# steineggerlab/unicore

Hardware: AMD Instinct MI355X
Metric: 3Di alignments/sec (cluster path) (higher is better)
Workload: dtype u16

## Files before the change

### include/unicore_cluster.h

```cpp
#ifndef UNICORE_CLUSTER_H
#define UNICORE_CLUSTER_H
#include <stddef.h>
#include <stdint.h>
#ifdef __cplusplus
extern "C" {
#endif

#define UC_OK 0
#define UC_ERR_GENERIC 1
#define UC_ERR_ARGS 2
#define UC_ERR_IO 3
#define UC_ERR_DEVICE 4

typedef struct uc_opts {
    uint32_t struct_size;
    int32_t threads;
    int32_t verbosity;
    int32_t device;
    int32_t num_gpus;
    const char *cluster_options;
    const char *data_dir;
} uc_opts;

#define UC_ABI_VERSION 9
// ... 103 lines not shown
#define UC_COMM_ID_BYTES 128
int uc_comm_unique_id(uint8_t id[UC_COMM_ID_BYTES]);
int uc_comm_create(const uint8_t id[UC_COMM_ID_BYTES], int32_t rank, int32_t world, int32_t device, uc_comm **out);
void uc_comm_destroy(uc_comm *c);
int uc_comm_info(const uc_comm *c, int32_t *nccl_ranks, int32_t *nccl_rank, int32_t *device);
int uc_engine_cluster_step(uc_engine *e, uc_comm *comm, int32_t target_shards, uint32_t *assign, uint64_t *n_alignments);

int uc_engine_align(uc_engine *e, uint32_t qbegin, uint32_t qend);
int uc_engine_alns_get(const uc_engine *e, uint32_t qbegin, uint32_t qend, uc_aln *out);
int uc_engine_edges_size(const uc_engine *e, uint64_t *n_edges);
int uc_engine_edges_get(const uc_engine *e, uint32_t *edges );

int uc_engine_stats(const uc_engine *e, uc_stats *out);
void uc_engine_reset_stats(uc_engine *e);
int uc_engine_td_onchip(const uc_engine *e, uint64_t *out );

int uc_engine_linclust_pairs(uc_engine *e, int32_t m, int32_t install, uint32_t *out_pairs, uint64_t cap, uint64_t *n_out);

int uc_setcover(uint32_t n, const uint32_t *edges, uint64_t n_edges, uint32_t *assign);
int uc_engine_setcover(uc_engine *e, const uint32_t *edges, uint64_t n_edges, uint32_t *assign);
int uc_cluster_graph(uint32_t n, const uint32_t *edges, uint64_t n_edges, const uint32_t *len, int32_t mode, uint32_t *assign);
int uc_engine_cluster_graph(uc_engine *e, int32_t mode, const uint32_t *edges, uint64_t n_edges, uint32_t *assign);
int uc_engine_reassign(uc_engine *e, const uint32_t *assign_in, uint32_t *assign_out, uint8_t *rejected_out, uint64_t counts[4]);
int uc_write_cluster_db(const char *out_cluster_db, uint32_t n, const uint32_t *assign);

#define UC_NO_GENE 0xffffffffu
int uc_profile_count(uint64_t n_rows, const uint32_t *group, const uint32_t *gene, uint32_t n_groups, uint32_t n_genes, const uint64_t *sp_off,
                     const uint32_t *sp, uint32_t n_species, uint32_t threshold, uint32_t *single, uint32_t *multiple, uint8_t *core,
                     uint64_t *core_off, uint32_t *core_gene, uint32_t *core_species, uint32_t *full);
int uc_profile_count_dev(int32_t device, uint64_t n_rows, const uint32_t *group, const uint32_t *gene, uint32_t n_groups, uint32_t n_genes,
// ... 114 lines not shown
```

### unicore_amd/__init__.py

```python
import ctypes as C
import os

import numpy as np

_HERE = os.path.dirname(os.path.abspath(__file__))
LIB_PATH = os.path.join(_HERE, "libunicore_cluster.so")

UC_OK, UC_ERR_GENERIC, UC_ERR_ARGS, UC_ERR_IO, UC_ERR_DEVICE = 0, 1, 2, 3, 4
NSTAGE = 8
PHASES = ("prefilter", "exchange_lists_to_home", "merge_at_home", "exchange_pairs_to_owner", "install_owned", "gapped", "edge_gather", "rank0_serial_cover")
STAGES = ("load", "index", "kmer", "ungapped", "select", "gapped", "setcover", "output")


class UcOpts(C.Structure):
    _fields_ = [("struct_size", C.c_uint32), ("threads", C.c_int32), ("verbosity", C.c_int32), ("device", C.c_int32),
                ("num_gpus", C.c_int32), ("cluster_options", C.c_char_p), ("data_dir", C.c_char_p)]


class UcStats(C.Structure):
    _fields_ = [(n, C.c_uint64) for n in (
        "n_seqs", "n_residues", "n_index_entries", "n_sim_kmers", "n_kmer_hits", "n_candidates", "n_prefilter_hits",
        "n_gapped_alignments", "n_start_alignments", "n_pk_reruns", "n_edges", "n_clusters", "cells_fwd", "cells_rev", "cells_start")] + [
        ("algorithmic_bytes", C.c_uint64 * NSTAGE), ("stage_seconds", C.c_double * NSTAGE),
        ("sw_kernel_ms", C.c_double), ("sw_kernel_launches", C.c_uint64), ("sw_algorithmic_bytes", C.c_uint64),
# ... 43 lines not shown
HIT_DTYPE = np.dtype([("target", "<u4"), ("score", "<i4"), ("diag", "<i4")])
ALN_DTYPE = np.dtype([(n, "<i4") for n in ("score", "score_rev", "corrected", "qstart", "qend", "tstart", "tend",
                                            "aln_len", "idents", "pass_evalue", "accepted", "gap_opens")])

SYMBOLS = (
    "uc_cluster", "uc_createtsv", "uc_rmdb", "uc_search", "uc_convertalis", "uc_last_error", "uc_version", "uc_check_options",
    "uc_option_arity", "uc_release_scratch", "uc_createdb", "uc_t5_load", "uc_t5_free", "uc_t5_encode", "uc_t5_get_stats", "uc_comm_unique_id", "uc_comm_create", "uc_comm_destroy", "uc_comm_info", "uc_engine_cluster_step",
    "uc_engine_create", "uc_engine_destroy", "uc_engine_load_db", "uc_engine_set_db", "uc_engine_num_seqs",
    "uc_engine_prefilter", "uc_engine_prefilter_range", "uc_engine_hits_size", "uc_engine_hits_get", "uc_engine_hits_get_range", "uc_engine_hits_set", "uc_engine_hits_merge",
    "uc_engine_hits_export_dev", "uc_engine_hits_import_dev", "uc_engine_setcover",
    "uc_hits_merge", "uc_engine_align", "uc_engine_alns_get", "uc_engine_edges_size", "uc_engine_edges_get",
    "uc_engine_stats", "uc_engine_reset_stats", "uc_setcover", "uc_write_cluster_db",
    "uc_engine_ungapped_batch", "uc_engine_ungapped_select", "uc_engine_ungapped_all", "uc_engine_sw_batch", "uc_engine_sw_pass", "uc_engine_sw_pass2", "uc_engine_backtraces_size", "uc_engine_backtraces_get",
    "uc_backtrace_render", "uc_format_output_check", "uc_engine_tb_emit_pass", "uc_abi_version", "uc_stats_size", "uc_set_round_hook",
    "uc_t5_gemm_variant", "uc_t5_kernel_gemm", "uc_t5_kernel_rmsnorm", "uc_t5_kernel_attention", "uc_t5_kernel_cnn_head", "uc_t5_bias_table",
    "uc_cluster_graph", "uc_engine_cluster_graph", "uc_engine_reassign", "uc_engine_td_onchip", "uc_engine_linclust_pairs",
    "uc_profile_count", "uc_profile_count_dev", "uc_profile",
    "uc_msa_center", "uc_msa_center_dev", "uc_msa_star", "uc_msa_star_dev", "uc_msa_filter", "uc_msa_filter_dev", "uc_tree",
    "uc_nj_counts", "uc_nj_counts_dev", "uc_nj_distances", "uc_nj_join", "uc_nj_join_dev", "uc_nj_newick", "uc_nj_geometry", "uc_tree_infer",
    "uc_nj_boot_columns", "uc_nj_boot_counts", "uc_nj_boot_counts_dev", "uc_nj_join_batch", "uc_nj_join_batch_dev", "uc_nj_support", "uc_nj_newick_support",
    "uc_nj_boot_geometry", "uc_tree_infer_boot",
)
NO_GENE = 0xFFFFFFFF
ABI_VERSION = 9
ROUND_HOOK = C.CFUNCTYPE(None, C.c_void_p, C.c_int32, C.c_uint32, C.POINTER(C.c_uint32), C.c_int32, C.c_void_p)

_lib = None


class UcError(RuntimeError):
    def __init__(self, code, msg):
# ... 45 lines not shown
    L.uc_engine_hits_get_range.argtypes = [vp, u32, u32, vp, vp]
    L.uc_engine_hits_set.argtypes = [vp, vp, vp]
    L.uc_engine_hits_merge.argtypes = [vp, C.c_int, C.POINTER(vp), C.POINTER(vp)]
    L.uc_engine_hits_export_dev.argtypes = [vp, vp, vp, vp, vp]
    L.uc_engine_setcover.argtypes = [vp, vp, u64, vp]
    L.uc_engine_hits_import_dev.argtypes = [vp, u64, vp, vp, vp, vp, u32, u32, C.POINTER(u64)]
    L.uc_hits_merge.argtypes = [u32, i32, C.c_int, C.POINTER(vp), C.POINTER(vp), vp, vp, u64, C.POINTER(u64)]
    L.uc_engine_align.argtypes = [vp, u32, u32]
    L.uc_engine_alns_get.argtypes = [vp, u32, u32, vp]
    L.uc_engine_edges_size.argtypes = [vp, C.POINTER(u64)]
    L.uc_engine_edges_get.argtypes = [vp, vp]
    L.uc_engine_stats.argtypes = [vp, C.POINTER(UcStats)]
    L.uc_engine_reset_stats.argtypes = [vp]
    L.uc_engine_reset_stats.restype = None
    L.uc_engine_td_onchip.argtypes = [vp, C.POINTER(C.c_uint64)]
    L.uc_engine_linclust_pairs.argtypes = [vp, i32, i32, vp, u64, C.POINTER(u64)]
    L.uc_setcover.argtypes = [u32, vp, u64, vp]
    L.uc_cluster_graph.argtypes = [u32, vp, u64, vp, i32, vp]
    L.uc_engine_cluster_graph.argtypes = [vp, i32, vp, u64, vp]
    L.uc_engine_reassign.argtypes = [vp, vp, vp, vp, vp]
    L.uc_write_cluster_db.argtypes = [C.c_char_p, u32, vp]
    L.uc_profile_count.argtypes = [u64, vp, vp, u32, u32, vp, vp, u32, u32] + [vp] * 7
    L.uc_profile_count_dev.argtypes = [i32, u64, vp, vp, u32, u32, vp, vp, u32, u32] + [vp] * 7
    L.uc_profile.argtypes = [C.c_char_p, C.c_char_p, C.c_char_p, u32, C.POINTER(UcOpts)]
    L.uc_msa_center.argtypes = [u32, vp, vp, vp]
    L.uc_msa_center_dev.argtypes = [i32, u32, vp, vp, vp]
    L.uc_msa_star.argtypes = [u32, vp, vp, u32] + [vp] * 8 + [vp, vp, vp, u64, vp, vp, u64, vp]
    L.uc_msa_star_dev.argtypes = [i32] + L.uc_msa_star.argtypes
    L.uc_msa_filter.argtypes = [u32, vp, vp, vp, u32, vp, vp, vp]
    L.uc_msa_filter_dev.argtypes = [i32] + L.uc_msa_filter.argtypes
# ... 655 lines not shown

    def edges(self):
        ne = C.c_uint64()
        _check(lib().uc_engine_edges_size(self._h, C.byref(ne)))
        e = np.zeros((max(ne.value, 1), 2), np.uint32)
        _check(lib().uc_engine_edges_get(self._h, e.ctypes.data))
        return e[: ne.value]

    def stats(self):
        st = UcStats()
        _check(lib().uc_engine_stats(self._h, C.byref(st)))
        d = st.as_dict()
        td = (C.c_uint64 * 4)()
        _check(lib().uc_engine_td_onchip(self._h, td))
        d["td_onchip_queries"], d["td_onchip_keys"] = int(td[0]), int(td[2])
        return d

    def reset_stats(self):
        lib().uc_engine_reset_stats(self._h)

    def ungapped(self, q, t, diag):
        q = np.ascontiguousarray(q, np.uint32); t = np.ascontiguousarray(t, np.uint32)
        diag = np.ascontiguousarray(diag, np.int32)
        out = np.zeros(len(q), np.int32)
        _check(lib().uc_engine_ungapped_batch(self._h, len(q), q.ctypes.data, t.ctypes.data, diag.ctypes.data, out.ctypes.data))
        return out

    def ungapped_select(self, q, t, diag, min_score):
        q = np.ascontiguousarray(q, np.uint32); t = np.ascontiguousarray(t, np.uint32)
        diag = np.ascontiguousarray(diag, np.int32)
# ... 66 lines not shown
```

### unicore_amd/csrc/uc_capi.cpp

```cpp
#include <sys/stat.h>

#include <algorithm>
#include <cmath>
#include <cstdlib>
#include <cstring>
#include <fstream>
#include <memory>

#include "uc_engine.h"
#include "uc_files.h"
#include "uc_multi.h"
#include "uc_t5.h"
#include "uc_workflow.h"

using namespace uc;

struct uc_comm {
    Comm c;
};
struct uc_t5 {
    T5Model m;
};

namespace {
// ... 316 lines not shown
        if (!h.empty()) { require(edges, "edges"); memcpy(edges, h.data(), h.size() * 4); }
    });
}

int uc_engine_stats(const uc_engine *e, uc_stats *out) {
    return guard([&] { require(e, "engine"); require(out, "out"); *out = e->e->stats; });
}

void uc_engine_reset_stats(uc_engine *e) {
    if (!e || !e->e) return;
    uc_stats &s = e->e->stats;
    const uint64_t ns = s.n_seqs, nr = s.n_residues;
    memset(&s, 0, sizeof s);
    s.n_seqs = ns; s.n_residues = nr;
    for (uint64_t &x : e->e->td_onchip) x = 0;
}

int uc_engine_td_onchip(const uc_engine *e, uint64_t *out) {
    return guard([&] { require(e, "engine"); require(out, "out"); for (int i = 0; i < 4; i++) out[i] = e->e->td_onchip[i]; });
}

int uc_engine_linclust_pairs(uc_engine *e, int32_t m, int32_t install, uint32_t *out_pairs, uint64_t cap, uint64_t *n_out) {
    return guard([&] {
        require(e, "engine"); require(n_out, "n_out");
        if (m > 1000) fail(UC_ERR_ARGS, "uc_engine_linclust_pairs: m must be <= 0 (the engine's --kmer-per-seq) or in [1,1000]");
        if (install != 0 && install != 1) fail(UC_ERR_ARGS, "uc_engine_linclust_pairs: install must be 0 or 1");
        if (cap && !install) require(out_pairs, "out_pairs");
        const int mo = m > 0 ? m : 0;
        if (install) { *n_out = e->e->linclust_hits(mo); return; }
        const std::vector<uint32_t> pr = e->e->linclust_pairs(mo);
// ... 460 lines not shown
```

### unicore_amd/csrc/uc_device.h

```cpp
#pragma once
#include <hip/hip_runtime.h>

#include <atomic>
#include <cstdint>

namespace uc {

struct PerDeviceOnce {
    std::atomic<uint64_t> mask{0};
    template <typename F>
    void operator()(F &&f) {
        int d = 0;
        (void)hipGetDevice(&d);
        const uint64_t bit = 1ull << (d & 63);
        if (!(mask.load(std::memory_order_acquire) & bit)) { f(); mask.fetch_or(bit, std::memory_order_release); }
    }
};

struct DeviceDb {
    uint32_t n = 0;
    const uint8_t *s3 = nullptr, *sa = nullptr;
    const uint16_t *lt = nullptr;
    const uint32_t *off = nullptr;
    const uint32_t *len = nullptr;
// ... 7 lines not shown

struct SwArgs {
    DeviceDb db;
    const SwTask *tasks;
    const uint32_t *pt;
    const int32_t *pqe, *pte;
    const int32_t *pqs = nullptr, *pts = nullptr;
    uint8_t *tbm = nullptr;
    const unsigned long long *tboff = nullptr;
    int tb_band = 0;
    const int32_t *pscore = nullptr;
    int32_t *oscore, *oqe, *ote;
    int open, ext;
    uint32_t tb_diag = 1u, tb_ident = 0u, tb_open = 1u, tb_ext = 1u;
    int32_t *oqe2 = nullptr, *ote2 = nullptr;
};

constexpr int SW_MAX_ROWS = 2048;

struct TbBand { int nl, dlo, dhi; };
__host__ __device__ inline TbBand tb_band_of(int qs, int qe, int tl, int G, int R, int W) {
    TbBand b;
    const int d0 = qs, d1 = qe - (tl - 1);
    b.dlo = (d0 < d1 ? d0 : d1) - W;
    b.dhi = (d0 < d1 ? d1 : d0) + W;
    const int nl = (b.dhi - b.dlo + R - 1) / (R + 1) + 1;
    b.nl = (W <= 0 || nl >= G) ? G : nl;
    return b;
}

// ... 14 lines not shown
__device__ __forceinline__ void block_add2(unsigned long long va, unsigned long long vb, T *da, T *db) {
    __shared__ unsigned long long part[2][16];
    for (int o = 32; o > 0; o >>= 1) { va += __shfl_down(va, o, 64); vb += __shfl_down(vb, o, 64); }
    if ((threadIdx.x & 63) == 0) { part[0][threadIdx.x >> 6] = va; part[1][threadIdx.x >> 6] = vb; }
    __syncthreads();
    if (threadIdx.x == 0) {
        unsigned long long sa = 0, sb = 0;
        for (uint32_t w = 0; w < (blockDim.x + 63) >> 6; w++) { sa += part[0][w]; sb += part[1][w]; }
        if (sa) atomicAdd(da, (T)sa);
        if (sb) atomicAdd(db, (T)sb);
    }
}
#endif

void launch_sw_class(int G, int R, int mode, const SwArgs &a, uint32_t n_tasks, hipStream_t s);
void launch_sw_pk_class(int G, int R, int mode, const SwArgs &a, uint32_t n_tasks, hipStream_t s);
constexpr uint32_t SW_LONG_TASK_PAIRS = 8;
size_t sw_long_work_ints(int mode, uint32_t n_pairs, uint32_t max_len, uint32_t *stride);
void launch_sw_long(int mode, const SwArgs &a, uint32_t n_tasks, uint32_t pair_base, int32_t *work, uint32_t stride, hipStream_t s);
void launch_ungapped(const DeviceDb &db, uint64_t n, const uint32_t *q, const uint32_t *t, const int32_t *diag,
                     int32_t *score, unsigned long long *overlap_sum , hipStream_t s);
void launch_comp_bias(const DeviceDb &db, int scale_milli, int8_t *out, hipStream_t s);
void launch_db_pad(uint32_t n, const uint32_t *off, const uint32_t *len, const uint32_t *cur ,
                   const uint64_t *roff, const uint8_t *r3, const uint8_t *ra,
                   uint64_t total, uint8_t *s3, uint8_t *sa, uint16_t *lt, hipStream_t s);

}
```

### unicore_amd/csrc/uc_engine.h

```cpp
#pragma once
#include <hip/hip_runtime.h>

#include <algorithm>
#include <atomic>
#include <chrono>
#include <cstdint>
#include <cstdio>
#include <cstdlib>
#include <memory>
#include <mutex>
#include <string>
#include <utility>
#include <vector>

#include "uc_common.h"
#include "uc_db.h"
#include "uc_device.h"
#include "uc_options.h"
#include "unicore_cluster.h"

namespace uc {

struct OomRelief { bool (*fn)(void *) = nullptr; void *ctx = nullptr; };
inline OomRelief &oom_relief_slot() { static thread_local OomRelief r; return r; }
// ... 215 lines not shown
    void clear_edges() { edges.clear(); n_edges_dev = 0; edges_on_host = true; }
    const std::vector<uint32_t> &host_edges();

    uc_stats stats{};

    explicit Engine(const Params &pp, int dev);
    ~Engine();
    void upload_db(bool keep_raw = false);
    void upload_sub_db(const std::vector<uint32_t> &cur, const std::vector<uint64_t> &full_off);
    uint64_t plan_db_layout();
    void finish_db_install(struct Timer &tm);
    void prefilter(uint32_t tbegin, uint32_t tend, uint32_t qbegin = 0, uint32_t qend = UINT32_MAX);
    void prefilter_cells(uint32_t tbegin, uint32_t tend, const std::vector<std::pair<uint32_t, uint32_t>> &others);
    PrefilterScratch *pre = nullptr;
    AlignScratch *aln = nullptr;
    uint64_t td_onchip[4] = {0, 0, 0, 0};
    uint64_t last_align_hits = 0;
    void drop_scratch();
    bool relieve_pressure(int stage);
    int stage_frames[3] = {0, 0, 0};
    struct PressureScope {
        OomRelief saved;
        struct Ctx { Engine *e; int stage; } ctx;
        PressureScope(Engine &E, int stage) : saved(oom_relief_slot()), ctx{&E, stage} {
            E.stage_frames[stage]++;
            oom_relief_slot() = OomRelief{[](void *c) { return ((Ctx *)c)->e->relieve_pressure(((Ctx *)c)->stage); }, &ctx};
        }
        ~PressureScope() { oom_relief_slot() = saved; ctx.e->stage_frames[ctx.stage]--; }
        PressureScope(const PressureScope &) = delete;
        PressureScope &operator=(const PressureScope &) = delete;
// ... 51 lines not shown
```

### unicore_amd/csrc/uc_sw.hip

```cpp
#include "uc_sw_impl.hpp"

namespace uc {

void launch_sw_class_m0(int G, int R, const SwArgs &a, uint32_t n_tasks, hipStream_t s);
void launch_sw_class_m1(int G, int R, const SwArgs &a, uint32_t n_tasks, hipStream_t s);
void launch_sw_class_m2(int G, int R, const SwArgs &a, uint32_t n_tasks, hipStream_t s);
void launch_sw_class_m3(int G, int R, const SwArgs &a, uint32_t n_tasks, hipStream_t s);

void launch_sw_class(int G, int R, int mode, const SwArgs &a, uint32_t n_tasks, hipStream_t s) {
    if (n_tasks == 0) return;
    if (mode == 0) launch_sw_class_m0(G, R, a, n_tasks, s);
    else if (mode == 1) launch_sw_class_m1(G, R, a, n_tasks, s);
    else if (mode == 2) launch_sw_class_m2(G, R, a, n_tasks, s);
    else launch_sw_class_m3(G, R, a, n_tasks, s);
}

void launch_sw_pk_class_m0(int G, int R, const SwArgs &a, uint32_t n_tasks, hipStream_t s);
void launch_sw_pk_class_m1(int G, int R, const SwArgs &a, uint32_t n_tasks, hipStream_t s);
void launch_sw_pk_class_m2(int G, int R, const SwArgs &a, uint32_t n_tasks, hipStream_t s);
void launch_sw_pk_class_m4(int G, int R, const SwArgs &a, uint32_t n_tasks, hipStream_t s);
void launch_sw_pk_class_m6(int G, int R, const SwArgs &a, uint32_t n_tasks, hipStream_t s);
void launch_sw_pk_class_m7(int G, int R, const SwArgs &a, uint32_t n_tasks, hipStream_t s);
void launch_sw_pk_class(int G, int R, int mode, const SwArgs &a, uint32_t n_tasks, hipStream_t s) {
    if (n_tasks == 0) return;
    if (mode == 0) launch_sw_pk_class_m0(G, R, a, n_tasks, s);
    else if (mode == 1) launch_sw_pk_class_m1(G, R, a, n_tasks, s);
    else if (mode == 2) launch_sw_pk_class_m2(G, R, a, n_tasks, s);
    else if (mode == 4) launch_sw_pk_class_m4(G, R, a, n_tasks, s);
    else if (mode == 6) launch_sw_pk_class_m6(G, R, a, n_tasks, s);
    else launch_sw_pk_class_m7(G, R, a, n_tasks, s);
}

__global__ void __launch_bounds__(256) db_pad_kernel(uint32_t n, const uint32_t *off, const uint32_t *len, const uint32_t *cur, const uint64_t *roff, const uint8_t *r3,
                                                     const uint8_t *ra, uint64_t total, uint8_t *s3, uint8_t *sa, uint16_t *lt) {
    for (uint64_t p = (uint64_t)blockIdx.x * 256 + threadIdx.x; p < total + 16; p += (uint64_t)gridDim.x * 256) {
        if (p < 16) { lt[p] = (uint16_t)SW_PADPACK; continue; }
        const uint64_t q = p - 16;
        uint8_t c3 = 20, ca = 20;
        uint16_t pair = (uint16_t)SW_PADPACK;
        if (n) {
            uint32_t lo = 0, hi = n;
            while (hi - lo > 1) {
                const uint32_t mid = lo + ((hi - lo) >> 1);
                if (off[mid] <= q) lo = mid; else hi = mid;
            }
// ... 121 lines not shown
```

### unicore_amd/csrc/uc_sw_pk_impl.hpp

```cpp
#pragma once
#include <hip/hip_runtime.h>

#include "uc_device.h"
#include "uc_sw_impl.hpp"

namespace uc {

constexpr int SW_PK_OVF = 0x7C00 - 256;

typedef uint16_t u16x2_t __attribute__((ext_vector_type(2)));
typedef uint32_t u32x4_u __attribute__((ext_vector_type(4), aligned(4)));
typedef uint32_t u32x2_u __attribute__((ext_vector_type(2), aligned(4)));
typedef const uint32_t __attribute__((address_space(4))) *sw_cu32p;
__device__ __forceinline__ u16x2_t pk_v(uint32_t x) { return __builtin_bit_cast(u16x2_t, x); }
__device__ __forceinline__ uint32_t pk_u(u16x2_t v) { return __builtin_bit_cast(uint32_t, v); }
__device__ __forceinline__ uint32_t pk_add_sat(uint32_t a, uint32_t b) { return pk_u(__builtin_elementwise_add_sat(pk_v(a), pk_v(b))); }
__device__ __forceinline__ uint32_t pk_sub_sat(uint32_t a, uint32_t b) { return pk_u(__builtin_elementwise_sub_sat(pk_v(a), pk_v(b))); }
__device__ __forceinline__ uint32_t pk_max(uint32_t a, uint32_t b) { return pk_u(__builtin_elementwise_max(pk_v(a), pk_v(b))); }
__device__ __forceinline__ uint32_t pk_min(uint32_t a, uint32_t b) {
    uint32_t r;
    asm("v_pk_min_u16 %0, %1, %2" : "=v"(r) : "v"(a), "v"(b));
    return r;
}
__device__ __forceinline__ uint32_t pk_max3(uint32_t a, uint32_t b, uint32_t c) {
    uint32_t r;
    asm("v_pk_maximum3_f16 %0, %1, %2, %3" : "=v"(r) : "v"(a), "v"(b), "v"(c));
    return r;
}

template <int G, int R, int MODE, int NW>
__global__ void __launch_bounds__(NW * 64) sw_pk_kernel(const SwArgs a) {
    constexpr bool TBB = MODE == 7;
    constexpr bool KNOWN = MODE == 4 || MODE == 6;
    constexpr int BASE = KNOWN ? MODE - 4 : (TBB ? 0 : MODE);
    constexpr bool TRACK = BASE != 1 && !TBB, MASK = BASE == 2 || TBB, REVQ = BASE != 0, REVT = BASE == 2;
    constexpr int RW = (R + 3) / 4, BW = RW | 1, RSW = G * BW, NT = NW * 64;
    static_assert(R % 2 == 0 && R <= 32, "R must be even, <= 32");
    extern __shared__ __attribute__((aligned(16))) uint32_t lds[];
    uint32_t *P3 = lds, *PA = lds + SW_NLET * RSW;
    uint32_t *slot_ctr = lds + 2 * SW_NLET * RSW;

    const SwTask task = a.tasks[blockIdx.x];
    const int tid = threadIdx.x, lane = tid & 63;
    const int g = lane % G;
    const uint32_t qoff = a.db.off[task.q];
    const int lq = (int)a.db.len[task.q];
    const uint32_t open2 = (uint32_t)a.open * 0x10001u, ext2 = (uint32_t)a.ext * 0x10001u, bias2 = 128u * 0x10001u;
    const uint32_t nslots = (task.count + 1) >> 1;

    for (int idx = tid; idx < SW_NLET * G * RW; idx += NT) {
        const int c = idx / (G * RW), rem = idx % (G * RW), gg = rem / RW, k = rem % RW;
        uint32_t w3 = 0, wa = 0;
#pragma unroll
        for (int b = 0; b < 4; b++) {
            const int row = gg * R + 4 * k + b;
            if (row < lq && c < 21 && 4 * k + b < R) {
                const int qi = REVQ ? lq - 1 - row : row;
                const int q3 = a.db.s3[qoff + qi], qa = a.db.sa[qoff + qi];
                w3 |= (uint32_t)(a.db.S3[q3 * 21 + c] + 64) << (8 * b);
                wa |= (uint32_t)(a.db.SA[qa * 21 + c] + 64) << (8 * b);
            }
        }
        P3[c * RSW + gg * BW + k] = w3;
        PA[c * RSW + gg * BW + k] = wa;
    }
    if (tid == 0) *slot_ctr = 0;
    __syncthreads();

    uint32_t H[R], E[R], rowbest[(TRACK && !KNOWN) ? R : 1];
    uint32_t mskA[MASK ? RW : 1], mskB[MASK ? RW : 1];
    uint32_t best = 0, Hlast = 0, prevHup = 0, fout = 0;
    int colA = -1, colB = -1;
    [[maybe_unused]] uint32_t knownA = 0, knownB = 0;
    [[maybe_unused]] int key2A = 0x7fffffff, key2B = 0x7fffffff;
    uint32_t gA = 0, gB = 0, toffA = 0, toffB = 0;
    [[maybe_unused]] unsigned long long tbA = 0, tbB = 0;
    [[maybe_unused]] int tsaA = 0, tsbA = 0, tsaB = 0, tsbB = 0;
    [[maybe_unused]] uint32_t trowA = 0, trowB = 0, tslotA = 0, tslotB = 0;
    int tlenA = 0, tlenB = 0, rowoffA = 0, rowoffB = 0;
    bool vB = false, active = false;
    int lst = 0, nst = 0;
    uint32_t c1 = 0, cin = 0;
// ... 34 lines not shown
    uint32_t off3 = (uint32_t)(g * BW) * 4u, offa = (uint32_t)(SW_NLET * RSW + g * BW) * 4u;
    asm volatile("" : "+v"(off3), "+v"(offa));
    auto fetch_profile = [&]() __attribute__((always_inline)) {
        const char *l8 = (const char *)lds;
        const uint32_t *pA3 = (const uint32_t *)(l8 + (cin & 0xff) * (RSW * 4) + off3), *pAa = (const uint32_t *)(l8 + ((cin >> 8) & 0xff) * (RSW * 4) + offa);
        const uint32_t *pB3 = (const uint32_t *)(l8 + ((cin >> 16) & 0xff) * (RSW * 4) + off3), *pBa = (const uint32_t *)(l8 + (cin >> 24) * (RSW * 4) + offa);
#pragma unroll
        for (int k = 0; k < RW; k++) { nA3[k] = pA3[k]; nAa[k] = pAa[k]; nB3[k] = pB3[k]; nBa[k] = pBa[k]; }
    };

    auto start_slot = [&]() {
        uint32_t idx = 0;
        if (g == 0) idx = atomicAdd(slot_ctr, 1u);
        if constexpr (G == 64) idx = (uint32_t)__builtin_amdgcn_readfirstlane((int)idx);
        else idx = (uint32_t)__shfl((int)idx, lane - g, 64);
        active = idx < nslots;
        if (!active) return;
        const uint32_t iA = 2 * idx, iB = iA + 1;
        vB = iB < task.count;
        gA = task.begin + iA;
        gB = task.begin + (vB ? iB : iA);
        const uint32_t tA = a.pt[gA], tB = a.pt[gB];
        toffA = a.db.off[tA]; toffB = a.db.off[tB];
        tlenA = REVT ? a.pte[gA] + 1 : (int)a.db.len[tA];
        tlenB = vB ? (REVT ? a.pte[gB] + 1 : (int)a.db.len[tB]) : 0;
        if constexpr (TBB) {
            toffA += (uint32_t)a.pts[gA]; toffB += (uint32_t)a.pts[gB];
            tlenA = a.pte[gA] - a.pts[gA] + 1;
            tlenB = vB ? a.pte[gB] - a.pts[gB] + 1 : 0;
            tbA = a.tboff[gA]; tbB = a.tboff[gB];
            const int qsA = a.pqs[gA], qeA = a.pqe[gA], qsB = a.pqs[gB], qeB = a.pqe[gB];
            {
                constexpr int RBc = 4 * RW;
                const TbBand bA = tb_band_of(qsA, qeA, tlenA, G, R, a.tb_band), bB = tb_band_of(qsB, qeB, vB ? tlenB : 1, G, R, a.tb_band);
                const bool fullA = bA.nl >= G, fullB = bB.nl >= G;
                tsaA = fullA ? 0 : g * (R + 1) - bA.dhi; tsbA = fullA ? 0x7fffffff : g * (R + 1) + R - 1 - bA.dlo;
// ... 1 lines not shown
                trowA = (uint32_t)(bA.nl * RBc); trowB = (uint32_t)(bB.nl * RBc);
                tslotA = (uint32_t)((g % bA.nl) * RBc); tslotB = (uint32_t)((g % bB.nl) * RBc);
            }
#pragma unroll
            for (int k = 0; k < RW; k++) {
                uint32_t ma = 0, mb = 0;
#pragma unroll
                for (int b = 0; b < 4; b++) {
                    const int row = g * R + 4 * k + b;
                    ma |= (row >= qsA && row <= qeA ? 0xFFu : 0u) << (8 * b);
                    mb |= (row >= qsB && row <= qeB ? 0xFFu : 0u) << (8 * b);
                }
                mskA[k] = ma; mskB[k] = mb;
            }
        } else if constexpr (MASK) {
            rowoffA = lq - 1 - a.pqe[gA];
            rowoffB = lq - 1 - a.pqe[gB];
#pragma unroll
            for (int k = 0; k < RW; k++) {
                uint32_t ma = 0, mb = 0;
#pragma unroll
                for (int b = 0; b < 4; b++) {
                    ma |= (g * R + 4 * k + b >= rowoffA ? 0xFFu : 0u) << (8 * b);
                    mb |= (g * R + 4 * k + b >= rowoffB ? 0xFFu : 0u) << (8 * b);
                }
                mskA[k] = ma; mskB[k] = mb;
            }
        }
        if constexpr (G != 64) {
            ltA = a.db.lt + toffA - (REVT ? 1 : 0);
            ltB = vB ? a.db.lt + toffB - (REVT ? 1 : 0) : a.db.lt + toffA - 1;
        }
// ... 192 lines not shown

    start_slot();
    while (__builtin_amdgcn_ballot_w64(active) != 0) {
        if (active) {
            do_step(lst, false);
            do_step(lst + 1, true);
            lst += 2;
            if (lst >= nst) {
                finish_slot();
                start_slot();
            }
        }
    }
}

template <int MODE>
void launch_sw_pk_class_mode(int G, int R, const SwArgs &a, uint32_t n_tasks, hipStream_t s) {
#define UC_SW_CASE(GG, RR)                                                                              \
    if (G == GG && R == RR) {                                                                           \
        constexpr int BW = (((RR + 3) / 4) | 1);                                                        \
         \
        constexpr int NW = GG == 16 ? 2 : (GG == 32 ? 4 : (RR < 14 ? 2 : 8));                           \
        const size_t lds = (size_t)2 * SW_NLET * GG * BW * 4 + 16;                                      \
        static PerDeviceOnce once;                                                                      \
        if (lds > 64 * 1024)                                                                            \
            once([&] { (void)hipFuncSetAttribute((const void *)sw_pk_kernel<GG, RR, MODE, NW>,           \
                                                 hipFuncAttributeMaxDynamicSharedMemorySize, (int)lds); }); \
        hipLaunchKernelGGL((sw_pk_kernel<GG, RR, MODE, NW>), dim3(n_tasks), dim3(NW * 64), lds, s, a);  \
        return;                                                                                         \
    }
    UC_SW_CASE(16, 2) UC_SW_CASE(16, 4) UC_SW_CASE(16, 6) UC_SW_CASE(16, 8) UC_SW_CASE(16, 10) UC_SW_CASE(16, 12)
    UC_SW_CASE(16, 14) UC_SW_CASE(16, 16) UC_SW_CASE(16, 18) UC_SW_CASE(16, 20) UC_SW_CASE(16, 22) UC_SW_CASE(16, 24)
    UC_SW_CASE(32, 14) UC_SW_CASE(32, 16) UC_SW_CASE(32, 18) UC_SW_CASE(32, 20) UC_SW_CASE(32, 22) UC_SW_CASE(32, 24)
    UC_SW_CASE(64, 14) UC_SW_CASE(64, 16) UC_SW_CASE(64, 18) UC_SW_CASE(64, 20) UC_SW_CASE(64, 22) UC_SW_CASE(64, 24)
    UC_SW_CASE(64, 26) UC_SW_CASE(64, 28) UC_SW_CASE(64, 30) UC_SW_CASE(64, 32)
    if constexpr (MODE == 4 || MODE == 6) {
        UC_SW_CASE(64, 2) UC_SW_CASE(64, 4) UC_SW_CASE(64, 6) UC_SW_CASE(64, 8) UC_SW_CASE(64, 10) UC_SW_CASE(64, 12)
    }
#undef UC_SW_CASE
    fprintf(stderr, "unicore-cluster: no packed SW kernel for class (G=%d, R=%d)\n", G, R);
    abort();
}

template <int MODE>
void preload_sw_pk_mode() {
    hipFuncAttributes fa;
    (void)hipFuncGetAttributes(&fa, (const void *)sw_pk_kernel<64, 14, MODE, 8>);
}

}
```

### unicore_amd/csrc/uc_sw_pk_m0.hip

```cpp
#include "uc_sw_pk_impl.hpp"
namespace uc {
void launch_sw_pk_class_m0(int G, int R, const SwArgs &a, uint32_t n_tasks, hipStream_t s) {
    launch_sw_pk_class_mode<0>(G, R, a, n_tasks, s);
}
void preload_sw_pk_m0() { preload_sw_pk_mode<0>(); }
}
```

### unicore_amd/csrc/uc_sw_pk_m1.hip

```cpp
#include "uc_sw_pk_impl.hpp"
namespace uc {
void launch_sw_pk_class_m1(int G, int R, const SwArgs &a, uint32_t n_tasks, hipStream_t s) {
    launch_sw_pk_class_mode<1>(G, R, a, n_tasks, s);
}
void preload_sw_pk_m1() { preload_sw_pk_mode<1>(); }
}
```

### unicore_amd/csrc/uc_sw_pk_m2.hip

```cpp
#include "uc_sw_pk_impl.hpp"
namespace uc {
void launch_sw_pk_class_m2(int G, int R, const SwArgs &a, uint32_t n_tasks, hipStream_t s) {
    launch_sw_pk_class_mode<2>(G, R, a, n_tasks, s);
}
}
```

### unicore_amd/csrc/uc_sw_pk_m4.hip

```cpp
#include "uc_sw_pk_impl.hpp"
namespace uc {
void launch_sw_pk_class_m4(int G, int R, const SwArgs &a, uint32_t n_tasks, hipStream_t s) {
    launch_sw_pk_class_mode<4>(G, R, a, n_tasks, s);
}
void preload_sw_pk_m4() { preload_sw_pk_mode<4>(); }
}
```

### unicore_amd/csrc/uc_sw_pk_m6.hip

```cpp
#include "uc_sw_pk_impl.hpp"
namespace uc {
void launch_sw_pk_class_m6(int G, int R, const SwArgs &a, uint32_t n_tasks, hipStream_t s) {
    launch_sw_pk_class_mode<6>(G, R, a, n_tasks, s);
}
void preload_sw_pk_m6() { preload_sw_pk_mode<6>(); }
}
```

### unicore_amd/csrc/uc_sw_pk_m7.hip

```cpp
#include "uc_sw_pk_impl.hpp"
namespace uc {
void launch_sw_pk_class_m7(int G, int R, const SwArgs &a, uint32_t n_tasks, hipStream_t s) {
    launch_sw_pk_class_mode<7>(G, R, a, n_tasks, s);
}
}
```

### unicore_amd/csrc/uc_sw_plan.hip

```cpp
#include <mutex>
#include <hip/hip_runtime.h>

#include <algorithm>
#include <cstdlib>
#include <cstring>

#include <rocprim/rocprim.hpp>

#include "uc_align_internal.h"

namespace uc {

const ClassTable h_tab[4] = {
    {16,
     {64, 128, 192, 256, 320, 384, 448, 512, 640, 768, 896, 1024, 1280, 1536, 1792, 2048},
     {16, 16, 16, 16, 16, 16, 16, 16, 32, 32, 32, 32, 64, 64, 64, 64},
     {4, 8, 12, 16, 20, 24, 28, 32, 20, 24, 28, 32, 20, 24, 28, 32},
     {0, 0, 0, 0, 0, 0, 0, 0, 0, 0, 0, 0, 0, 0, 0, 0},
     {256, 256, 256, 256, 256, 256, 256, 256, 64, 64, 64, 64, 24, 24, 24, 24}},
    {28,
     {32, 64, 96, 128, 160, 192, 224, 256, 288, 320, 352, 384, 448, 512, 576, 640, 704, 768, 896, 1024, 1152, 1280, 1408, 1536, 1664, 1792, 1920, 2048},
     {16, 16, 16, 16, 16, 16, 16, 16, 16, 16, 16, 16, 32, 32, 32, 32, 32, 32, 64, 64, 64, 64, 64, 64, 64, 64, 64, 64},
     {2, 4, 6, 8, 10, 12, 14, 16, 18, 20, 22, 24, 14, 16, 18, 20, 22, 24, 14, 16, 18, 20, 22, 24, 26, 28, 30, 32},
     {1, 1, 1, 1, 1, 1, 1, 1, 1, 1, 1, 1, 1, 1, 1, 1, 1, 1, 1, 1, 1, 1, 1, 1, 1, 1, 1, 1},
// ... 259 lines not shown
        if (gaps_out) gaps_out[p] = (int32_t)gaps;
    }
}

struct MaxU32 {
    __host__ __device__ uint32_t operator()(uint32_t a, uint32_t b) const { return a > b ? a : b; }
};

}

int pk_known_tab(uint32_t n_pairs, uint32_t n_queries) {
    static const bool on = !(getenv("UC_SW_SPARSE") && atoi(getenv("UC_SW_SPARSE")) == 0);
    return on && (double)n_pairs < 2.5 * (double)n_queries ? 3 : 1;
}

void max_scan_u32(Engine &E, DevBuf<char> &tmp, const uint32_t *in, uint32_t *out, uint32_t n) {
    rocprim_call(tmp, [&](void *t, size_t &b) { return rocprim::inclusive_scan(t, b, in, out, (size_t)n, MaxU32(), E.stream); });
}

uint32_t compact(Engine &E, DevBuf<char> &tmp, const uint32_t *flag, uint32_t *pos, uint32_t n) {
    rocprim_call(tmp, [&](void *t, size_t &b) { return rocprim::exclusive_scan(t, b, flag, pos, 0u, (size_t)n, rocprim::plus<uint32_t>(), E.stream); });
    if (!n) return 0;
    uint32_t a = 0, b = 0;
    UC_HIP(hipMemcpyAsync(&a, pos + (n - 1), 4, hipMemcpyDeviceToHost, E.stream));
    UC_HIP(hipMemcpyAsync(&b, flag + (n - 1), 4, hipMemcpyDeviceToHost, E.stream));
    UC_HIP(hipStreamSynchronize(E.stream));
    return a + b;
}

PackedPrefix packed_prefix(const SwPlan &P) {
// ... 92 lines not shown
        SwArgs al = a;
        al.tasks = P.tasks.p + P.task_base[tab.n];
        launch_sw_long(imode, al, P.task_base[tab.n + 1] - P.task_base[tab.n], gb, work.p, long_stride, E.stream);
        UC_HIP(hipGetLastError());
        slot++;
        launches++;
    }
    for (int c = tab.n - 1; c >= 0 && !only_long; c--) {
        const uint32_t c0 = std::max(P.task_base[c], t0), c1 = std::min(P.task_base[c + 1], t1);
        if (c0 >= c1) continue;
        const uint32_t nt = c1 - c0;
        SwArgs ac = a;
        ac.tasks = P.tasks.p + c0;
        hipStream_t st = slot % E.n_streams == 0 ? E.stream : E.aux[slot % E.n_streams - 1];
        slot++;
        if (tab.pk[c]) launch_sw_pk_class(tab.G[c], tab.R[c], mode, ac, nt, st);
        else launch_sw_class(tab.G[c], tab.R[c], imode, ac, nt, st);
        UC_HIP(hipGetLastError());
        launches++;
    }
    for (int i = 0; i < E.n_streams - 1; i++) {
        UC_HIP(hipEventRecord(E.ev_join[i], E.aux[i]));
        UC_HIP(hipStreamWaitEvent(E.stream, E.ev_join[i], 0));
    }
    return launches;
}

__global__ void __launch_bounds__(256) pk_flag_kernel(uint32_t n_pk, const int32_t *os, const int32_t *oqe, int ovf, int ovf_only, uint32_t *flag) {
    for (uint32_t i = blockIdx.x * 256 + threadIdx.x; i < n_pk; i += gridDim.x * 256)
        flag[i] = (os[i] >= ovf || (!ovf_only && oqe && oqe[i] == -2)) ? 1u : 0u;
}
__global__ void __launch_bounds__(256) pk_gather_kernel(uint32_t n_pk, const uint32_t *flag, const uint32_t *pos, const uint32_t *sq,
// ... 96 lines not shown
```

Baseline: 23.13 million.

## Pack two small packed-SW query tasks per workgroup with sorted slot scheduling

```diff
diff --git a/include/unicore_cluster.h b/include/unicore_cluster.h
--- a/include/unicore_cluster.h
+++ b/include/unicore_cluster.h
@@ -141,6 +141,7 @@
 int uc_engine_stats(const uc_engine *e, uc_stats *out);
 void uc_engine_reset_stats(uc_engine *e);
 int uc_engine_td_onchip(const uc_engine *e, uint64_t *out );
+int uc_engine_sw_task_queries(const uc_engine *e, uint64_t *out );
 
 int uc_engine_linclust_pairs(uc_engine *e, int32_t m, int32_t install, uint32_t *out_pairs, uint64_t cap, uint64_t *n_out);
 
diff --git a/unicore_amd/__init__.py b/unicore_amd/__init__.py
--- a/unicore_amd/__init__.py
+++ b/unicore_amd/__init__.py
@@ -81,7 +81,7 @@
     "uc_engine_ungapped_batch", "uc_engine_ungapped_select", "uc_engine_ungapped_all", "uc_engine_sw_batch", "uc_engine_sw_pass", "uc_engine_sw_pass2", "uc_engine_backtraces_size", "uc_engine_backtraces_get",
     "uc_backtrace_render", "uc_format_output_check", "uc_engine_tb_emit_pass", "uc_abi_version", "uc_stats_size", "uc_set_round_hook",
     "uc_t5_gemm_variant", "uc_t5_kernel_gemm", "uc_t5_kernel_rmsnorm", "uc_t5_kernel_attention", "uc_t5_kernel_cnn_head", "uc_t5_bias_table",
-    "uc_cluster_graph", "uc_engine_cluster_graph", "uc_engine_reassign", "uc_engine_td_onchip", "uc_engine_linclust_pairs",
+    "uc_cluster_graph", "uc_engine_cluster_graph", "uc_engine_reassign", "uc_engine_td_onchip", "uc_engine_sw_task_queries", "uc_engine_linclust_pairs",
     "uc_profile_count", "uc_profile_count_dev", "uc_profile",
     "uc_msa_center", "uc_msa_center_dev", "uc_msa_star", "uc_msa_star_dev", "uc_msa_filter", "uc_msa_filter_dev", "uc_tree",
     "uc_nj_counts", "uc_nj_counts_dev", "uc_nj_distances", "uc_nj_join", "uc_nj_join_dev", "uc_nj_newick", "uc_nj_geometry", "uc_tree_infer",
@@ -157,6 +157,7 @@
     L.uc_engine_reset_stats.argtypes = [vp]
     L.uc_engine_reset_stats.restype = None
     L.uc_engine_td_onchip.argtypes = [vp, C.POINTER(C.c_uint64)]
+    L.uc_engine_sw_task_queries.argtypes = [vp, C.POINTER(C.c_uint64)]
     L.uc_engine_linclust_pairs.argtypes = [vp, i32, i32, vp, u64, C.POINTER(u64)]
     L.uc_setcover.argtypes = [u32, vp, u64, vp]
     L.uc_cluster_graph.argtypes = [u32, vp, u64, vp, i32, vp]
@@ -842,6 +843,9 @@
         td = (C.c_uint64 * 4)()
         _check(lib().uc_engine_td_onchip(self._h, td))
         d["td_onchip_queries"], d["td_onchip_keys"] = int(td[0]), int(td[2])
+        mq = (C.c_uint64 * 2)()
+        _check(lib().uc_engine_sw_task_queries(self._h, mq))
+        d["sw_multiquery_launches"], d["sw_multiquery_tasks"] = int(mq[0]), int(mq[1])
         return d
 
     def reset_stats(self):
diff --git a/unicore_amd/csrc/uc_capi.cpp b/unicore_amd/csrc/uc_capi.cpp
--- a/unicore_amd/csrc/uc_capi.cpp
+++ b/unicore_amd/csrc/uc_capi.cpp
@@ -354,6 +354,11 @@
     memset(&s, 0, sizeof s);
     s.n_seqs = ns; s.n_residues = nr;
     for (uint64_t &x : e->e->td_onchip) x = 0;
+    for (uint64_t &x : e->e->sw_task_queries) x = 0;
+}
+
+int uc_engine_sw_task_queries(const uc_engine *e, uint64_t *out) {
+    return guard([&] { require(e, "engine"); require(out, "out"); for (int i = 0; i < 2; i++) out[i] = e->e->sw_task_queries[i]; });
 }
 
 int uc_engine_td_onchip(const uc_engine *e, uint64_t *out) {
diff --git a/unicore_amd/csrc/uc_device.h b/unicore_amd/csrc/uc_device.h
--- a/unicore_amd/csrc/uc_device.h
+++ b/unicore_amd/csrc/uc_device.h
@@ -45,6 +45,7 @@
     int open, ext;
     uint32_t tb_diag = 1u, tb_ident = 0u, tb_open = 1u, tb_ext = 1u;
     int32_t *oqe2 = nullptr, *ote2 = nullptr;
+    uint32_t n_tasks = 0;
 };
 
 constexpr int SW_MAX_ROWS = 2048;
@@ -89,7 +90,7 @@
 #endif
 
 void launch_sw_class(int G, int R, int mode, const SwArgs &a, uint32_t n_tasks, hipStream_t s);
-void launch_sw_pk_class(int G, int R, int mode, const SwArgs &a, uint32_t n_tasks, hipStream_t s);
+int launch_sw_pk_class(int G, int R, int mode, const SwArgs &a, uint32_t n_tasks, hipStream_t s, int kmax = 1, uint32_t tcap = 0);
 constexpr uint32_t SW_LONG_TASK_PAIRS = 8;
 size_t sw_long_work_ints(int mode, uint32_t n_pairs, uint32_t max_len, uint32_t *stride);
 void launch_sw_long(int mode, const SwArgs &a, uint32_t n_tasks, uint32_t pair_base, int32_t *work, uint32_t stride, hipStream_t s);
diff --git a/unicore_amd/csrc/uc_engine.h b/unicore_amd/csrc/uc_engine.h
--- a/unicore_amd/csrc/uc_engine.h
+++ b/unicore_amd/csrc/uc_engine.h
@@ -253,6 +253,7 @@
     void prefilter_cells(uint32_t tbegin, uint32_t tend, const std::vector<std::pair<uint32_t, uint32_t>> &others);
     PrefilterScratch *pre = nullptr;
     AlignScratch *aln = nullptr;
+    uint64_t sw_task_queries[2] = {0, 0};
     uint64_t td_onchip[4] = {0, 0, 0, 0};
     uint64_t last_align_hits = 0;
     void drop_scratch();
diff --git a/unicore_amd/csrc/uc_sw.hip b/unicore_amd/csrc/uc_sw.hip
--- a/unicore_amd/csrc/uc_sw.hip
+++ b/unicore_amd/csrc/uc_sw.hip
@@ -15,20 +15,20 @@
     else launch_sw_class_m3(G, R, a, n_tasks, s);
 }
 
-void launch_sw_pk_class_m0(int G, int R, const SwArgs &a, uint32_t n_tasks, hipStream_t s);
-void launch_sw_pk_class_m1(int G, int R, const SwArgs &a, uint32_t n_tasks, hipStream_t s);
-void launch_sw_pk_class_m2(int G, int R, const SwArgs &a, uint32_t n_tasks, hipStream_t s);
-void launch_sw_pk_class_m4(int G, int R, const SwArgs &a, uint32_t n_tasks, hipStream_t s);
-void launch_sw_pk_class_m6(int G, int R, const SwArgs &a, uint32_t n_tasks, hipStream_t s);
-void launch_sw_pk_class_m7(int G, int R, const SwArgs &a, uint32_t n_tasks, hipStream_t s);
-void launch_sw_pk_class(int G, int R, int mode, const SwArgs &a, uint32_t n_tasks, hipStream_t s) {
-    if (n_tasks == 0) return;
-    if (mode == 0) launch_sw_pk_class_m0(G, R, a, n_tasks, s);
-    else if (mode == 1) launch_sw_pk_class_m1(G, R, a, n_tasks, s);
-    else if (mode == 2) launch_sw_pk_class_m2(G, R, a, n_tasks, s);
-    else if (mode == 4) launch_sw_pk_class_m4(G, R, a, n_tasks, s);
-    else if (mode == 6) launch_sw_pk_class_m6(G, R, a, n_tasks, s);
-    else launch_sw_pk_class_m7(G, R, a, n_tasks, s);
+int launch_sw_pk_class_m0(int G, int R, const SwArgs &a, uint32_t n_tasks, hipStream_t s, int kmax, uint32_t tcap);
+int launch_sw_pk_class_m1(int G, int R, const SwArgs &a, uint32_t n_tasks, hipStream_t s, int kmax, uint32_t tcap);
+int launch_sw_pk_class_m2(int G, int R, const SwArgs &a, uint32_t n_tasks, hipStream_t s, int kmax, uint32_t tcap);
+int launch_sw_pk_class_m4(int G, int R, const SwArgs &a, uint32_t n_tasks, hipStream_t s, int kmax, uint32_t tcap);
+int launch_sw_pk_class_m6(int G, int R, const SwArgs &a, uint32_t n_tasks, hipStream_t s, int kmax, uint32_t tcap);
+int launch_sw_pk_class_m7(int G, int R, const SwArgs &a, uint32_t n_tasks, hipStream_t s, int kmax, uint32_t tcap);
+int launch_sw_pk_class(int G, int R, int mode, const SwArgs &a, uint32_t n_tasks, hipStream_t s, int kmax, uint32_t tcap) {
+    if (n_tasks == 0) return 1;
+    if (mode == 0) return launch_sw_pk_class_m0(G, R, a, n_tasks, s, kmax, tcap);
+    if (mode == 1) return launch_sw_pk_class_m1(G, R, a, n_tasks, s, kmax, tcap);
+    if (mode == 2) return launch_sw_pk_class_m2(G, R, a, n_tasks, s, kmax, tcap);
+    if (mode == 4) return launch_sw_pk_class_m4(G, R, a, n_tasks, s, kmax, tcap);
+    if (mode == 6) return launch_sw_pk_class_m6(G, R, a, n_tasks, s, kmax, tcap);
+    return launch_sw_pk_class_m7(G, R, a, n_tasks, s, kmax, tcap);
 }
 
 __global__ void __launch_bounds__(256) db_pad_kernel(uint32_t n, const uint32_t *off, const uint32_t *len, const uint32_t *cur, const uint64_t *roff, const uint8_t *r3,
diff --git a/unicore_amd/csrc/uc_sw_pk_impl.hpp b/unicore_amd/csrc/uc_sw_pk_impl.hpp
--- a/unicore_amd/csrc/uc_sw_pk_impl.hpp
+++ b/unicore_amd/csrc/uc_sw_pk_impl.hpp
@@ -28,7 +28,9 @@
     return r;
 }
 
-template <int G, int R, int MODE, int NW>
+constexpr int SW_MQ_SLOTS = 128;
+
+template <int G, int R, int MODE, int NW, int K = 1>
 __global__ void __launch_bounds__(NW * 64) sw_pk_kernel(const SwArgs a) {
     constexpr bool TBB = MODE == 7;
     constexpr bool KNOWN = MODE == 4 || MODE == 6;
@@ -37,10 +39,14 @@
     constexpr int RW = (R + 3) / 4, BW = RW | 1, RSW = G * BW, NT = NW * 64;
     static_assert(R % 2 == 0 && R <= 32, "R must be even, <= 32");
     extern __shared__ __attribute__((aligned(16))) uint32_t lds[];
+    static_assert(K == 1 || (K <= 4 && G < 64 && !TBB), "several tasks per workgroup: G < 64, not MODE 7");
+    constexpr int PB = 2 * SW_NLET * RSW;
     uint32_t *P3 = lds, *PA = lds + SW_NLET * RSW;
-    uint32_t *slot_ctr = lds + 2 * SW_NLET * RSW;
-
-    const SwTask task = a.tasks[blockIdx.x];
+    uint32_t *slot_ctr = lds + K * PB;
+    [[maybe_unused]] uint32_t *tinfo = slot_ctr + 4, *sstep = tinfo + 4 * K;
+    [[maybe_unused]] uint8_t *stab = (uint8_t *)(sstep + SW_MQ_SLOTS);
+
+    const SwTask task = a.tasks[K * blockIdx.x];
     const int tid = threadIdx.x, lane = tid & 63;
     const int g = lane % G;
     const uint32_t qoff = a.db.off[task.q];
@@ -64,8 +70,68 @@
         P3[c * RSW + gg * BW + k] = w3;
         PA[c * RSW + gg * BW + k] = wa;
     }
+    if constexpr (K > 1) {
+        const uint32_t task0 = (uint32_t)K * blockIdx.x, nk = min((uint32_t)K, a.n_tasks - task0);
+        uint32_t base[K + 1];
+        base[0] = 0; base[1] = nslots;
+        if (tid == 0) { tinfo[0] = task.begin; tinfo[1] = task.count; tinfo[2] = (uint32_t)lq; }
+#pragma unroll
+        for (int t = 1; t < K; t++) {
+            base[t + 1] = base[t];
+            if ((uint32_t)t < nk) {
+                const SwTask tk = a.tasks[task0 + t];
+                const uint32_t qofft = a.db.off[tk.q];
+                const int lqt = (int)a.db.len[tk.q];
+                for (int idx = tid; idx < SW_NLET * G * RW; idx += NT) {
+                    const int c = idx / (G * RW), rem = idx % (G * RW), gg = rem / RW, k = rem % RW;
+                    uint32_t w3 = 0, wa = 0;
+#pragma unroll
+                    for (int b = 0; b < 4; b++) {
+                        const int row = gg * R + 4 * k + b;
+                        if (row < lqt && c < 21 && 4 * k + b < R) {
+                            const int qi = REVQ ? lqt - 1 - row : row;
+                            const int q3 = a.db.s3[qofft + qi], qa = a.db.sa[qofft + qi];
+                            w3 |= (uint32_t)(a.db.S3[q3 * 21 + c] + 64) << (8 * b);
+                            wa |= (uint32_t)(a.db.SA[qa * 21 + c] + 64) << (8 * b);
+                        }
+                    }
+                    P3[t * PB + c * RSW + gg * BW + k] = w3;
+                    PA[t * PB + c * RSW + gg * BW + k] = wa;
+                }
+                base[t + 1] += (tk.count + 1) >> 1;
+                if (tid == 0) { tinfo[4 * t] = tk.begin; tinfo[4 * t + 1] = tk.count; tinfo[4 * t + 2] = (uint32_t)lqt; }
+            }
+        }
+        const uint32_t mq_slots = min(base[K], (uint32_t)SW_MQ_SLOTS);
+        if (tid == 0) tinfo[3] = mq_slots;
+        for (uint32_t e = tid; e < mq_slots; e += NT) {
+            uint32_t t = 0;
+#pragma unroll
+            for (int j = 1; j < K; j++) t += e >= base[j] ? 1u : 0u;
+            uint32_t eb = 0;
+#pragma unroll
+            for (int j = 1; j < K; j++) eb = t == (uint32_t)j ? base[j] : eb;
+            const SwTask tk = a.tasks[task0 + t];
+            const uint32_t i = e - eb, pA = tk.begin + 2 * i, pB = pA + (2 * i + 1 < tk.count ? 1u : 0u);
+            const int la = REVT ? a.pte[pA] + 1 : (int)a.db.len[a.pt[pA]], lb = REVT ? a.pte[pB] + 1 : (int)a.db.len[a.pt[pB]];
+            sstep[e] = ((uint32_t)((max(la, lb) + G) & ~1) << 8) | (t << 6) | i;
+        }
+    }
     if (tid == 0) *slot_ctr = 0;
     __syncthreads();
+    if constexpr (K > 1) {
+        const uint32_t mq_slots = tinfo[3];
+        for (uint32_t e = tid; e < mq_slots; e += NT) {
+            const uint32_t v = sstep[e], s = v >> 8;
+            uint32_t rank = 0;
+            for (uint32_t j = 0; j < mq_slots; j++) {
+                const uint32_t sj = sstep[j] >> 8;
+                rank += (sj > s || (sj == s && j < e)) ? 1u : 0u;
+            }
+            stab[rank] = (uint8_t)(v & 0xffu);
+        }
+        __syncthreads();
+    }
 
     uint32_t H[R], E[R], rowbest[(TRACK && !KNOWN) ? R : 1];
     uint32_t mskA[MASK ? RW : 1], mskB[MASK ? RW : 1];
@@ -130,12 +196,22 @@
         if (g == 0) idx = atomicAdd(slot_ctr, 1u);
         if constexpr (G == 64) idx = (uint32_t)__builtin_amdgcn_readfirstlane((int)idx);
         else idx = (uint32_t)__shfl((int)idx, lane - g, 64);
-        active = idx < nslots;
+        if constexpr (K == 1) active = idx < nslots;
+        else active = idx < tinfo[3];
         if (!active) return;
+        [[maybe_unused]] uint32_t mq_begin = 0, mq_count = 0;
+        [[maybe_unused]] int mq_lq = 0;
+        if constexpr (K > 1) {
+            const uint32_t code = stab[idx], t = code >> 6;
+            idx = code & 63u;
+            mq_begin = tinfo[4 * t]; mq_count = tinfo[4 * t + 1]; mq_lq = (int)tinfo[4 * t + 2];
+            off3 = (t * PB + (uint32_t)(g * BW)) * 4u;
+            offa = off3 + (uint32_t)(SW_NLET * RSW) * 4u;
+        }
         const uint32_t iA = 2 * idx, iB = iA + 1;
-        vB = iB < task.count;
-        gA = task.begin + iA;
-        gB = task.begin + (vB ? iB : iA);
+        vB = iB < (K == 1 ? task.count : mq_count);
+        gA = (K == 1 ? task.begin : mq_begin) + iA;
+        gB = (K == 1 ? task.begin : mq_begin) + (vB ? iB : iA);
         const uint32_t tA = a.pt[gA], tB = a.pt[gB];
         toffA = a.db.off[tA]; toffB = a.db.off[tB];
         tlenA = REVT ? a.pte[gA] + 1 : (int)a.db.len[tA];
@@ -167,8 +243,8 @@
                 mskA[k] = ma; mskB[k] = mb;
             }
         } else if constexpr (MASK) {
-            rowoffA = lq - 1 - a.pqe[gA];
-            rowoffB = lq - 1 - a.pqe[gB];
+            rowoffA = (K == 1 ? lq : mq_lq) - 1 - a.pqe[gA];
+            rowoffB = (K == 1 ? lq : mq_lq) - 1 - a.pqe[gB];
 #pragma unroll
             for (int k = 0; k < RW; k++) {
                 uint32_t ma = 0, mb = 0;
@@ -391,20 +467,38 @@
     }
 }
 
+constexpr int sw_pk_class_queries(int G, int R, int mode) {
+    if (G != 16 || R < 4) return 1;
+    if (mode == 4) return (R == 8 || R == 10 || R == 14) ? 1 : 2;
+    return (mode == 0 || mode == 1 || mode == 6) ? 2 : 1;
+}
+
 template <int MODE>
-void launch_sw_pk_class_mode(int G, int R, const SwArgs &a, uint32_t n_tasks, hipStream_t s) {
+int launch_sw_pk_class_mode(int G, int R, const SwArgs &a, uint32_t n_tasks, hipStream_t s, int kmax, uint32_t tcap) {
+#define UC_SW_LAUNCH(GG, RR, NW, KK)                                                                    \
+    {                                                                                                   \
+        const size_t lds = (size_t)KK * 2 * SW_NLET * GG * BW * 4 + 16 + (KK > 1 ? 16 * KK + 5 * SW_MQ_SLOTS : 0); \
+        static PerDeviceOnce once;                                                                      \
+        if (lds > 64 * 1024)                                                                            \
+            once([&] { (void)hipFuncSetAttribute((const void *)sw_pk_kernel<GG, RR, MODE, NW, KK>,       \
+                                                 hipFuncAttributeMaxDynamicSharedMemorySize, (int)lds); }); \
+        SwArgs ak = a;                                                                                  \
+        ak.n_tasks = n_tasks;                                                                           \
+        hipLaunchKernelGGL((sw_pk_kernel<GG, RR, MODE, NW, KK>), dim3((n_tasks + KK - 1) / KK), dim3(NW * 64), lds, s, ak); \
+        return KK;                                                                                      \
+    }
 #define UC_SW_CASE(GG, RR)                                                                              \
     if (G == GG && R == RR) {                                                                           \
         constexpr int BW = (((RR + 3) / 4) | 1);                                                        \
          \
         constexpr int NW = GG == 16 ? 2 : (GG == 32 ? 4 : (RR < 14 ? 2 : 8));                           \
-        const size_t lds = (size_t)2 * SW_NLET * GG * BW * 4 + 16;                                      \
-        static PerDeviceOnce once;                                                                      \
-        if (lds > 64 * 1024)                                                                            \
-            once([&] { (void)hipFuncSetAttribute((const void *)sw_pk_kernel<GG, RR, MODE, NW>,           \
-                                                 hipFuncAttributeMaxDynamicSharedMemorySize, (int)lds); }); \
-        hipLaunchKernelGGL((sw_pk_kernel<GG, RR, MODE, NW>), dim3(n_tasks), dim3(NW * 64), lds, s, a);  \
-        return;                                                                                         \
+        constexpr int KC = sw_pk_class_queries(GG, RR, MODE);                                           \
+        if constexpr (KC > 1) {                                                                         \
+            const uint32_t ts = (tcap + 1) / 2;                             \
+             \
+            if (kmax > 1 && ts <= 64 && KC * ts <= (uint32_t)SW_MQ_SLOTS) UC_SW_LAUNCH(GG, RR, NW * KC, KC) \
+        }                                                                                               \
+        UC_SW_LAUNCH(GG, RR, NW, 1)                                                                     \
     }
     UC_SW_CASE(16, 2) UC_SW_CASE(16, 4) UC_SW_CASE(16, 6) UC_SW_CASE(16, 8) UC_SW_CASE(16, 10) UC_SW_CASE(16, 12)
     UC_SW_CASE(16, 14) UC_SW_CASE(16, 16) UC_SW_CASE(16, 18) UC_SW_CASE(16, 20) UC_SW_CASE(16, 22) UC_SW_CASE(16, 24)
@@ -415,6 +509,7 @@
         UC_SW_CASE(64, 2) UC_SW_CASE(64, 4) UC_SW_CASE(64, 6) UC_SW_CASE(64, 8) UC_SW_CASE(64, 10) UC_SW_CASE(64, 12)
     }
 #undef UC_SW_CASE
+#undef UC_SW_LAUNCH
     fprintf(stderr, "unicore-cluster: no packed SW kernel for class (G=%d, R=%d)\n", G, R);
     abort();
 }
diff --git a/unicore_amd/csrc/uc_sw_pk_m0.hip b/unicore_amd/csrc/uc_sw_pk_m0.hip
--- a/unicore_amd/csrc/uc_sw_pk_m0.hip
+++ b/unicore_amd/csrc/uc_sw_pk_m0.hip
@@ -1,7 +1,7 @@
 #include "uc_sw_pk_impl.hpp"
 namespace uc {
-void launch_sw_pk_class_m0(int G, int R, const SwArgs &a, uint32_t n_tasks, hipStream_t s) {
-    launch_sw_pk_class_mode<0>(G, R, a, n_tasks, s);
+int launch_sw_pk_class_m0(int G, int R, const SwArgs &a, uint32_t n_tasks, hipStream_t s, int kmax, uint32_t tcap) {
+    return launch_sw_pk_class_mode<0>(G, R, a, n_tasks, s, kmax, tcap);
 }
 void preload_sw_pk_m0() { preload_sw_pk_mode<0>(); }
 }
diff --git a/unicore_amd/csrc/uc_sw_pk_m1.hip b/unicore_amd/csrc/uc_sw_pk_m1.hip
--- a/unicore_amd/csrc/uc_sw_pk_m1.hip
+++ b/unicore_amd/csrc/uc_sw_pk_m1.hip
@@ -1,7 +1,7 @@
 #include "uc_sw_pk_impl.hpp"
 namespace uc {
-void launch_sw_pk_class_m1(int G, int R, const SwArgs &a, uint32_t n_tasks, hipStream_t s) {
-    launch_sw_pk_class_mode<1>(G, R, a, n_tasks, s);
+int launch_sw_pk_class_m1(int G, int R, const SwArgs &a, uint32_t n_tasks, hipStream_t s, int kmax, uint32_t tcap) {
+    return launch_sw_pk_class_mode<1>(G, R, a, n_tasks, s, kmax, tcap);
 }
 void preload_sw_pk_m1() { preload_sw_pk_mode<1>(); }
 }
diff --git a/unicore_amd/csrc/uc_sw_pk_m2.hip b/unicore_amd/csrc/uc_sw_pk_m2.hip
--- a/unicore_amd/csrc/uc_sw_pk_m2.hip
+++ b/unicore_amd/csrc/uc_sw_pk_m2.hip
@@ -1,6 +1,6 @@
 #include "uc_sw_pk_impl.hpp"
 namespace uc {
-void launch_sw_pk_class_m2(int G, int R, const SwArgs &a, uint32_t n_tasks, hipStream_t s) {
-    launch_sw_pk_class_mode<2>(G, R, a, n_tasks, s);
+int launch_sw_pk_class_m2(int G, int R, const SwArgs &a, uint32_t n_tasks, hipStream_t s, int kmax, uint32_t tcap) {
+    return launch_sw_pk_class_mode<2>(G, R, a, n_tasks, s, kmax, tcap);
 }
 }
diff --git a/unicore_amd/csrc/uc_sw_pk_m4.hip b/unicore_amd/csrc/uc_sw_pk_m4.hip
--- a/unicore_amd/csrc/uc_sw_pk_m4.hip
+++ b/unicore_amd/csrc/uc_sw_pk_m4.hip
@@ -1,7 +1,7 @@
 #include "uc_sw_pk_impl.hpp"
 namespace uc {
-void launch_sw_pk_class_m4(int G, int R, const SwArgs &a, uint32_t n_tasks, hipStream_t s) {
-    launch_sw_pk_class_mode<4>(G, R, a, n_tasks, s);
+int launch_sw_pk_class_m4(int G, int R, const SwArgs &a, uint32_t n_tasks, hipStream_t s, int kmax, uint32_t tcap) {
+    return launch_sw_pk_class_mode<4>(G, R, a, n_tasks, s, kmax, tcap);
 }
 void preload_sw_pk_m4() { preload_sw_pk_mode<4>(); }
 }
diff --git a/unicore_amd/csrc/uc_sw_pk_m6.hip b/unicore_amd/csrc/uc_sw_pk_m6.hip
--- a/unicore_amd/csrc/uc_sw_pk_m6.hip
+++ b/unicore_amd/csrc/uc_sw_pk_m6.hip
@@ -1,7 +1,7 @@
 #include "uc_sw_pk_impl.hpp"
 namespace uc {
-void launch_sw_pk_class_m6(int G, int R, const SwArgs &a, uint32_t n_tasks, hipStream_t s) {
-    launch_sw_pk_class_mode<6>(G, R, a, n_tasks, s);
+int launch_sw_pk_class_m6(int G, int R, const SwArgs &a, uint32_t n_tasks, hipStream_t s, int kmax, uint32_t tcap) {
+    return launch_sw_pk_class_mode<6>(G, R, a, n_tasks, s, kmax, tcap);
 }
 void preload_sw_pk_m6() { preload_sw_pk_mode<6>(); }
 }
diff --git a/unicore_amd/csrc/uc_sw_pk_m7.hip b/unicore_amd/csrc/uc_sw_pk_m7.hip
--- a/unicore_amd/csrc/uc_sw_pk_m7.hip
+++ b/unicore_amd/csrc/uc_sw_pk_m7.hip
@@ -1,6 +1,6 @@
 #include "uc_sw_pk_impl.hpp"
 namespace uc {
-void launch_sw_pk_class_m7(int G, int R, const SwArgs &a, uint32_t n_tasks, hipStream_t s) {
-    launch_sw_pk_class_mode<7>(G, R, a, n_tasks, s);
+int launch_sw_pk_class_m7(int G, int R, const SwArgs &a, uint32_t n_tasks, hipStream_t s, int kmax, uint32_t tcap) {
+    return launch_sw_pk_class_mode<7>(G, R, a, n_tasks, s, kmax, tcap);
 }
 }
diff --git a/unicore_amd/csrc/uc_sw_plan.hip b/unicore_amd/csrc/uc_sw_plan.hip
--- a/unicore_amd/csrc/uc_sw_plan.hip
+++ b/unicore_amd/csrc/uc_sw_plan.hip
@@ -297,6 +297,14 @@
     return on && (double)n_pairs < 2.5 * (double)n_queries ? 3 : 1;
 }
 
+static double sw_task_queries_slots() {
+    static const double v = [] {
+        if (getenv("UC_SW_TASK_QUERIES") && atoi(getenv("UC_SW_TASK_QUERIES")) == 1) return 0.0;
+        return getenv("UC_SW_TASK_SLOTS") ? atof(getenv("UC_SW_TASK_SLOTS")) : 24.0;
+    }();
+    return v;
+}
+
 void max_scan_u32(Engine &E, DevBuf<char> &tmp, const uint32_t *in, uint32_t *out, uint32_t n) {
     rocprim_call(tmp, [&](void *t, size_t &b) { return rocprim::inclusive_scan(t, b, in, out, (size_t)n, MaxU32(), E.stream); });
 }
@@ -419,8 +427,11 @@
         ac.tasks = P.tasks.p + c0;
         hipStream_t st = slot % E.n_streams == 0 ? E.stream : E.aux[slot % E.n_streams - 1];
         slot++;
-        if (tab.pk[c]) launch_sw_pk_class(tab.G[c], tab.R[c], mode, ac, nt, st);
-        else launch_sw_class(tab.G[c], tab.R[c], imode, ac, nt, st);
+        if (tab.pk[c]) {
+            const double slots = 0.5 * (double)(P.pair_base[c + 1] - P.pair_base[c]) / (double)(P.task_base[c + 1] - P.task_base[c]);
+            const int k = launch_sw_pk_class(tab.G[c], tab.R[c], mode, ac, nt, st, slots < sw_task_queries_slots() ? 2 : 1, tab.tcap[c]);
+            if (k > 1) { E.sw_task_queries[0]++; E.sw_task_queries[1] += nt; }
+        } else launch_sw_class(tab.G[c], tab.R[c], imode, ac, nt, st);
         UC_HIP(hipGetLastError());
         launches++;
     }
```

Measured after the change: 23.48 million (median of 6 runs). 1.02x the previous value.
